# kylegrover/raymarch-algo-compare

Measured on AMD Instinct MI355X. Metric: Mrays/sec (mean iters/ray alongside), 1920x1080 Mandelbulb/Standard, higher is better.
Workload: dtype f64

## Files before the change

raymarch_algo_compare_amd/csrc/rm_capi.hip:

```cpp
#include <hip/hip_runtime.h>
#include <dlfcn.h>
#include <link.h>
#include <rccl/rccl.h>

#include <algorithm>
#include <cstdarg>
#include <cstdio>
#include <cstdlib>
#include <cstring>
#include <map>
#include <memory>
#include <mutex>
#include <optional>
#include <string>
#include <vector>

#include "../../include/rm_hip.h"
#include "rm_kernels.h"
#include "rm_launch_plan.h"
#include "rm_pipeline.h"
#include "rm_scene_program.h"
#include "rm_interval.h"
#include "rm_interval_catalogue.h"
#include "rm_segment.h"
// ... 89 lines not shown
        if (p) (void)hipFree(p);
        p = nullptr; cap = 0;
        hipError_t e = hipMalloc(&p, bytes);
        if (e != hipSuccess) return fail(RM_E_HIP, "hipMalloc(%zu) failed: %s", bytes, hipGetErrorString(e));
        cap = bytes;
        return RM_OK;
    }
    void release()
    {
        if (p) (void)hipFree(p);
        p = nullptr; cap = 0;
    }
};

void release_all(Buf* owner)
{
    for (Buf* b = owner; b; b = b->next) b->release();
}
Buf* g_workspace_bufs = nullptr;
Buf* g_comm_bufs = nullptr;
struct WsBuf : Buf { WsBuf() : Buf(g_workspace_bufs) {} };
struct CommBuf : Buf { CommBuf() : Buf(g_comm_bufs) {} };

struct Session {
    bool ready = false;
    int device = -1;
    hipStream_t stream = nullptr;
    hipDeviceProp_t prop;
    bool stats_ready = false;
    long long cost_key[10] = { -1 };
    bool cost_valid = false;
    hipEvent_t ev[2 * RM_MAX_TIMED];
    bool events = false;
    bool tracing = false;
    size_t trace_pix = 0;
    unsigned long long trace_t0 = 0;
    long long corder_key[12] = { -1 };
    bool corder_valid = false;
    bool pass_timing = false;
    hipEvent_t pev[RM_MAX_PASSES + 1];
    bool pev_ready = false;
    int pass_count = 0;
    bool last_was_pipeline = false;
    const unsigned long long* last_stats = nullptr;
    float long_marks[4] = { 0.f, 0.f, 0.f, 0.f };
    float last_push_ms = 0.f, last_pop_ms = 0.f;
    uint32_t generation = 0;
    struct QueueKey { int stride = 0; int writer = 0; size_t used = 0; } qkey[rm::kQueues];
    hipEvent_t frame_ev = nullptr;
    hipStream_t frame_stream = nullptr;
    bool frame_ev_valid = false;
    hipStream_t team_stream = nullptr;
    hipEvent_t split_ev[2] = { nullptr, nullptr };
};

struct State : Session {
    WsBuf stats, depth, iters, hit, traw, fs, bvar, evals, tcost, torder, queue[rm::kQueues];
    WsBuf in[2], out[4];
    WsBuf bstats;
    WsBuf ivprog;
    WsBuf ctl;
    WsBuf busy;
    WsBuf trace, trace_start, trace_detach;
    WsBuf ccost, corder;
    WsBuf ssim_depth, ssim_normal, ssim_color, ssim_hit;
    WsBuf ssim_ref, ssim_part, ssim_ssd, ssim_out;
    WsBuf score_depth, score_normal, score_hit, score_caps;
    WsBuf score_band, score_keys, score_small, score_part;
    WsBuf cap_out[5], cap_cams;
} g;

std::mutex g_mu;

struct Program {
    std::unique_ptr<rm::ProgramImage> img;
    void* dev = nullptr;
    double lipschitz = 1.0;
    bool ext = false;
};
std::mutex g_prog_mu;
std::map<int32_t, Program> g_programs;
int32_t g_next_program = RM_SCENE_PROGRAM_BASE;

bool is_program_id(int id) { return id >= RM_SCENE_PROGRAM_BASE; }

const rm::SceneLaunchers* program_launchers(bool ext)
{
#if defined(RM_DEV_STRATEGIES)
    if (ext) return rm::scene_launchers_program_ext ? rm::scene_launchers_program_ext() : nullptr;
    return rm::scene_launchers_program ? rm::scene_launchers_program() : nullptr;
#else
    return ext ? rm::scene_launchers_program_ext() : rm::scene_launchers_program();
#endif
}

bool program_exists(int id, bool* ext = nullptr)
{
    std::lock_guard<std::mutex> lk(g_prog_mu);
    auto it = g_programs.find(id);
    if (it == g_programs.end()) return false;
    if (ext) *ext = it->second.ext;
    return true;
}

const rm::SceneLaunchers* launchers(int id)
{
// ... 189 lines not shown
    if (d->tile_rows != 0 && d->tile_rows != 4 && d->tile_rows != 1) return fail(RM_E_BAD_ARG, "tile_rows must be 0, 4 or 1");
    if (d->tile_order_mode < 0 || d->tile_order_mode > 4) return fail(RM_E_BAD_ARG, "tile_order_mode must be 0 .. 4");
    if (d->eval_mode < 0 || d->eval_mode > 2) return fail(RM_E_BAD_ARG, "eval_mode must be 0, 1 or 2");
    if (d->resume_mode < 0 || d->resume_mode > 3) return fail(RM_E_BAD_ARG, "resume_mode must be 0..3");
    if (d->resume_grid < 0) return fail(RM_E_BAD_ARG, "negative resume_grid");
    if (d->pipeline < 0 || d->pipeline > 2) return fail(RM_E_BAD_ARG, "pipeline must be 0, 1 or 2");
    if (d->pipeline_form < 0 || d->pipeline_form > 3) return fail(RM_E_BAD_ARG, "pipeline_form must be 0 .. 3");
    if (d->team_grid < 0 || d->queue_first < 0 || d->queue_first > 3 || d->team_steal < 0 || d->team_steal > 2 ||
        d->queue_refill_min < 0 || d->queue_refill_min > 64 || d->queue_retry < 0 || d->team_retry < 0 || d->age_priority < 0)
        return fail(RM_E_BAD_ARG, "bad single-launch tuning field");
    if (d->exit_backlog < 0 || d->late_teams > 65536) return fail(RM_E_BAD_ARG, "bad late-team field");
    if (d->keep_busy > (1 << 20)) return fail(RM_E_BAD_ARG, "keep_busy out of range");
    if (d->early_handover > (1 << 20)) return fail(RM_E_BAD_ARG, "early_handover out of range");
    if (d->early_trips < 0 || d->early_trips > 64) return fail(RM_E_BAD_ARG, "early_trips out of range");
    if (d->band_rows < 0 || d->band_stride < 0 || d->band_offset < 0) return fail(RM_E_BAD_ARG, "negative band parameter");
    if (d->band_rows > 0 && d->band_stride > 1) {
        const int th = d->tile_rows ? d->tile_rows : 4;
        if (d->band_rows % th) return fail(RM_E_BAD_ARG, "band_rows must be a multiple of the tile height %d", th);
        if (d->band_offset >= d->band_stride) return fail(RM_E_BAD_ARG, "band_offset must be < band_stride");
        if (d->rows > 0) {
            const long long y = d->rows - 1;
            const long long last = d->row0 + ((y / d->band_rows) * d->band_stride + d->band_offset) * d->band_rows + y % d->band_rows;
            if (last >= d->height) return fail(RM_E_BAD_DIMS, "band-cyclic slice maps row %lld beyond height %d", last, d->height);
        }
    }
    return RM_OK;
}

rm::MarchCfg to_cfg(const RmMarchConfig& m)
{
    rm::MarchCfg c;
    c.hit_threshold = m.hit_threshold;
    c.max_distance = m.max_distance;
    c.lipschitz = m.lipschitz;
    c.max_iterations = m.max_iterations;
    c.full = m.full ? 1 : 0;
    c.prm = rm::default_strat_params();
    if (m.use_params) {
        static_assert(sizeof(RmStrategyParams) == sizeof(rm::StratParams), "RmStrategyParams and rm::StratParams must match");
        memcpy(&c.prm, &m.params, sizeof c.prm);
    }
    return c;
}

rm::LaunchPlan plan_for(const RmFrameDesc* d, int batch_frames = 0, const RmMarchConfig* configs = nullptr)
{
    const rm::SceneLaunchers* const sc = launchers(d->scene_id);
    const int strategy = d->strategy_id;
    rm::DeviceFacts f;
    f.cus = g.prop.multiProcessorCount;
    f.has_teams = sc->has_teams;
    f.has_resume_team = sc->resume_team != nullptr;
    f.entry_bytes = sc->entry_bytes(strategy);
    f.per_cu = [sc, strategy](rm::OccKernel k, int , int interleave, int batch) {
        int n = 0;
        const hipError_t e = k == rm::OccKernel::pipeline ? sc->occupancy_pipeline(strategy, interleave, batch, &n)
                                                          : sc->occupancy(strategy, interleave, batch, &n);
        return e == hipSuccess ? n : 0;
    };
    return rm::plan_launch(*d, f, batch_frames, configs);
}

rm::CameraParams camera_of(const double* cam14)
{
    rm::CameraParams c;
    for (int i = 0; i < 14; ++i) c.v[i] = cam14[i];
    return c;
}

int make_args(const RmFrameDesc* d, const rm::LaunchPlan& p, float* depth, int32_t* iters, uint8_t* hit, double* traw, double* fs,
              long long* bvar, unsigned long long* stats, rm::KernelArgs* a)
{
    memset(a, 0, sizeof *a);
    if (int rc = scene_data(d->scene_id, &a->scene_data)) return rc;
    a->single.cam = camera_of(d->cam);
    a->single.cfg = to_cfg(d->march);
    a->frames = nullptr;
    a->nframes = 1;
    a->full = d->march.full ? 1 : 0;
    a->width = d->width; a->height = d->height; a->row0 = d->row0; a->rows = d->rows;
    a->tiles_x = p.tiles_x;
    a->tiles_y = p.tiles_y;
    a->tiles_per_frame = a->tiles_x * a->tiles_y;
    a->tile_h = p.tile_h;
    a->refill_min = p.refill_min;
    a->hist_bins = rm::kHistBins;
    a->interleave = p.interleave;
    a->age_prio = d->age_priority > 0 ? d->age_priority : 0;
    if (d->band_rows > 0 && d->band_stride > 1) {
        a->band_rows = d->band_rows; a->band_stride = d->band_stride; a->band_offset = d->band_offset;
    }
    a->depth = depth; a->iters = iters; a->hit = hit; a->t_raw = traw; a->final_sdf = fs;
    a->block_var = bvar; a->stats = stats;
    a->fused_reduce = p.fused_reduce;
    if (p.park[0] > 0) {
        a->suspend_after = p.park[0];
        a->suspend_queue = 0;
    }
    if (p.single) {
        a->team_wgs = p.team_wgs;
        a->producer_waves = p.producer_waves;
        a->late_team_first = p.late_team_first;
        a->early_exit_wgs = p.early_exit_wgs;
        a->exit_backlog = p.exit_backlog;
        a->keep_busy = p.keep_busy;
        a->early_trips = p.early_trips;
        a->early_handover = p.early_handover;
        a->suspend_after2 = p.suspend_after2;
        a->q0_detach = p.q0_detach;
        a->q0_first = p.q0_first;
        a->q0_refill_min = p.q0_refill_min;
        a->q0_retry = p.q0_retry;
        a->team_retry = p.team_retry;
        a->team_steal = p.team_steal;
        a->max_spins = p.max_spins;
        a->team_prio = p.team_prio;
    }
    return RM_OK;
}

__global__ __launch_bounds__(1024) void order_tiles_kernel(const int32_t* __restrict__ cost, int32_t* __restrict__ order, int n)
{
    constexpr int BINS = 1024;
    __shared__ int hist[BINS];
    for (int b = threadIdx.x; b < BINS; b += blockDim.x) hist[b] = 0;
    __syncthreads();
    for (int i = threadIdx.x; i < n; i += blockDim.x) atomicAdd(&hist[min(max(cost[i], 0), BINS - 1)], 1);
    __syncthreads();
    if (threadIdx.x == 0) {
        int run = 0;
        for (int b = BINS - 1; b >= 0; --b) { const int c = hist[b]; hist[b] = run; run += c; }
    }
    __syncthreads();
    for (int i = threadIdx.x; i < n; i += blockDim.x) {
        const int pos = atomicAdd(&hist[min(max(cost[i], 0), BINS - 1)], 1);
        order[pos] = i;
    }
}

__global__ void center_cost_kernel(int32_t* __restrict__ cost, int tiles_x, int tiles_y, int nframes, int tile_h, int width, int height,
                                   int row0, int band_rows, int band_stride, int band_offset, float xweight)
{
    const int t = blockIdx.x * blockDim.x + threadIdx.x;
    if (t >= tiles_x * tiles_y * nframes) return;
    const int tf = t % (tiles_x * tiles_y);
    const int tx = tf % tiles_x, ty = tf / tiles_x;
    const int y0 = ty * tile_h;
    const int gy = band_rows > 0 ? row0 + ((y0 / band_rows) * band_stride + band_offset) * band_rows + (y0 % band_rows) : row0 + y0;
    const float cx = (tx * 64 + 32 - 0.5f * width) / (0.5f * height);
    const float cy = (gy + 0.5f * tile_h - 0.5f * height) / (0.5f * height);
    const float r = sqrtf(xweight * cx * cx + cy * cy);
    cost[t] = max(0, 1023 - (int)(r * 256.0f));
}

__global__ void block_var_kernel(const int32_t* __restrict__ iters, int width, int rows, int nframes,
                                 long long* __restrict__ out)
{
    const int bw = width >> 3, bh = rows >> 2;
    const long long n = (long long)bw * bh * nframes;
    const long long b = (long long)blockIdx.x * blockDim.x + threadIdx.x;
    if (b >= n) return;
    const int f = (int)(b / ((long long)bw * bh));
    const int r = (int)(b - (long long)f * bw * bh);
    const int by = r / bw, bx = r - by * bw;
    const int32_t* p = iters + (size_t)f * (size_t)rows * (size_t)width + (size_t)(by * 4) * (size_t)width + (size_t)(bx * 8);
    long long S = 0, Q = 0;
#pragma unroll
    for (int y = 0; y < 4; ++y)
#pragma unroll
// ... 447 lines not shown

}

extern "C" {

const char* rm_last_error(void) { return g_err; }
int rm_num_scenes(void) { return RM_NUM_SCENES; }

int rm_scene_program_create(const RmSceneOp* ops, int32_t nops, double lipschitz, int32_t* scene_id)
{
    if (!scene_id) return fail(RM_E_BAD_ARG, "scene_id is NULL");
    if (!(lipschitz > 0.0) || !(lipschitz - lipschitz == 0.0)) return fail(RM_E_BAD_ARG, "lipschitz must be finite and > 0");
    std::unique_ptr<rm::ProgramImage> img(new rm::ProgramImage());
    char why[256];
    if (!rm::program_encode(ops, nops, img.get(), why, sizeof why)) return fail(RM_E_BAD_ARG, "scene program: %s", why);
    std::lock_guard<std::mutex> lk(g_prog_mu);
    if (g_next_program == INT32_MAX) return fail(RM_E_BAD_ARG, "scene program ids exhausted");
    const int32_t id = g_next_program++;
    Program& p = g_programs[id];
    p.ext = rm::program_has_ext(*img);
    p.img = std::move(img);
    p.lipschitz = lipschitz;
    *scene_id = id;
    return RM_OK;
}

int rm_scene_program_destroy(int32_t scene_id)
{
    std::lock_guard<std::mutex> lk(g_mu);
    void* dev = nullptr;
    {
        std::lock_guard<std::mutex> lp(g_prog_mu);
        auto it = g_programs.find(scene_id);
        if (it == g_programs.end()) return no_such_program(scene_id);
        dev = it->second.dev;
        g_programs.erase(it);
    }
    if (dev) {
        if (g.ready) (void)hipSetDevice(g.device);
        HIP_TRY(hipFree(dev));
    }
    return RM_OK;
}
int rm_num_strategies(void) { return RM_NUM_STRATEGIES; }

void rm_default_strategy_params(RmStrategyParams* out)
{
    if (!out) return;
    const rm::StratParams p = rm::default_strat_params();
    memcpy(out, &p, sizeof *out);
}
size_t rm_stats_device_bytes(void) { return kStatsBytes; }

int rm_init(int device_id)
{
    std::lock_guard<std::mutex> lk(g_mu);
    if (g.ready && g.device == device_id) return RM_OK;
    if (g.ready) return fail(RM_E_BAD_ARG, "already initialised on device %d; call rm_shutdown() first", g.device);
    int n = 0;
    hipError_t e = hipGetDeviceCount(&n);
    if (e != hipSuccess || n <= 0)
        return fail(RM_E_NO_DEVICE, "no HIP device available (%s)", e == hipSuccess ? "count = 0" : hipGetErrorString(e));
    if (device_id < 0 || device_id >= n) return fail(RM_E_NO_DEVICE, "device %d out of range (have %d)", device_id, n);
    HIP_TRY(hipSetDevice(device_id));
    HIP_TRY(hipGetDeviceProperties(&g.prop, device_id));
    if (strncmp(g.prop.gcnArchName, "gfx950", 6) != 0)
        return fail(RM_E_NO_DEVICE, "device %d is %s; this library carries gfx950 code only", device_id, g.prop.gcnArchName);
    HIP_TRY(hipStreamCreateWithFlags(&g.stream, hipStreamNonBlocking));
    int rc = g.stats.ensure(kStatsBytes);
    if (rc) return rc;
    g.device = device_id;
    g.ready = true;
    return RM_OK;
}

void rm_shutdown(void)
{
    std::lock_guard<std::mutex> lk(g_mu);
    if (!g.ready) return;
    (void)hipSetDevice(g.device);
    (void)hipStreamSynchronize(g.stream);
    if (g.team_stream) {
        (void)hipStreamSynchronize(g.team_stream);
        for (auto& e : g.split_ev) (void)hipEventDestroy(e);
        (void)hipStreamDestroy(g.team_stream);
    }
    for (void* s : g_own_streams) {
        (void)hipStreamSynchronize((hipStream_t)s);
        (void)hipStreamDestroy((hipStream_t)s);
    }
    g_own_streams.clear();
    g_seen_streams.clear();
    release_all(g_workspace_bufs);
    if (g.frame_ev_valid) (void)hipEventDestroy(g.frame_ev);
    if (g.events) for (auto& e : g.ev) (void)hipEventDestroy(e);
    if (g.pev_ready) for (auto& e : g.pev) (void)hipEventDestroy(e);
    {
        std::lock_guard<std::mutex> lp(g_prog_mu);
        for (auto& kv : g_programs)
            if (kv.second.dev) {
                (void)hipFree(kv.second.dev);
                kv.second.dev = nullptr;
            }
    }
    (void)hipStreamDestroy(g.stream);
    static_cast<Session&>(g) = Session();
}

int rm_device_info(RmDeviceInfo* out)
{
    int rc = check_ready();
    if (rc) return rc;
    if (!out) return fail(RM_E_BAD_ARG, "out is NULL");
    memset(out, 0, sizeof *out);
    snprintf(out->name, sizeof out->name, "%s", g.prop.name);
    snprintf(out->arch, sizeof out->arch, "%s", g.prop.gcnArchName);
    out->device_id = g.device;
    out->compute_units = g.prop.multiProcessorCount;
    out->clock_mhz = g.prop.clockRate / 1000;
    out->wavefront_size = g.prop.warpSize;
    out->total_mem_bytes = g.prop.totalGlobalMem;
    return RM_OK;
}
// ... 1190 lines not shown
```

raymarch_algo_compare_amd/csrc/rm_kernels.h:

```cpp
#pragma once

#define RM_TABLES_IN_LDS 1

#include <hip/hip_runtime.h>
#include <stdint.h>
#include <type_traits>

#include "rm_camera.h"
#include "rm_capture.h"
#include "rm_scenes.h"
#include "rm_shape.h"
#include "rm_strategies.h"

namespace rm {

constexpr int kHistBins = 544;
constexpr int kStatsHead = 24;
constexpr int kStatsWords = kStatsHead + kHistBins;
constexpr int kQueues = 2;
constexpr int kStatsParts = 64;
constexpr int kStatsBlocks = 1 + kStatsParts;

struct FrameParams {
    CameraParams cam;
// ... 20 lines not shown
}


struct KernelArgs {
    FrameParams single;
    const FrameParams* frames;
    int32_t nframes;
    int32_t tiles_per_frame;
    int32_t full;
    int32_t width, height, row0, rows;
    int32_t tiles_x, tiles_y;
    int32_t tile_h;
    int32_t refill_min;
    int32_t interleave;
    int32_t hist_bins;
    int32_t band_rows, band_stride, band_offset;
    float* depth;
    int32_t* iters;
    uint8_t* hit;
    double* t_raw;
    int32_t* evals;
    double* final_sdf;
    int32_t raw_outputs;
    int32_t fused_reduce;
    long long* block_var;
    unsigned long long* stats;
    int32_t suspend_after, suspend_queue, queue_cap, queue_stride;
    unsigned char* queue[kQueues];
    const int32_t* tile_order;
    int32_t* tile_cost;
    unsigned long long* ctl;
    int32_t team_wgs, producer_waves;
    uint32_t generation;
    int32_t suspend_after2;
    int32_t q0_first;
    int32_t q0_detach;
    int32_t q0_refill_min;
    int32_t q0_retry;
    int32_t team_retry;
    int32_t team_steal;
    int32_t max_spins;
    int32_t team_prio;
    int32_t age_prio;
    int32_t marks;
    int32_t early_handover;
    int32_t early_trips;
    int32_t keep_busy;
    int32_t late_team_first, early_exit_wgs, exit_backlog;
    uint32_t* trace;
    uint32_t trace_cap;
    uint32_t* trace_start;
    uint32_t* trace_detach;
    const void* scene_data;
};

__device__ __forceinline__ int lane_id() { return (int)__builtin_amdgcn_mbcnt_hi(~0u, __builtin_amdgcn_mbcnt_lo(~0u, 0u)); }
__device__ __forceinline__ int rank_in_mask(unsigned long long m)
{
    return (int)__builtin_amdgcn_mbcnt_hi((unsigned)(m >> 32), __builtin_amdgcn_mbcnt_lo((unsigned)m, 0u));
}

__device__ __forceinline__ void store_raw(const KernelArgs& a, uint32_t gi, const Result& r, int nev)
{
    if (a.t_raw) a.t_raw[gi] = r.t;
#ifdef RM_DEV_STAMP
    if (a.evals) a.evals[gi] = (int)(__builtin_amdgcn_s_memrealtime() & 0x3fffffffull);
#else
    if (a.final_sdf) a.final_sdf[gi] = r.final_sdf;
    if (a.evals) a.evals[gi] = nev;
#endif
}

__device__ __forceinline__ void keep_busy_until(const unsigned long long* done, unsigned long long target, int burst)
{
    const unsigned long long t0 = __builtin_amdgcn_s_memrealtime();
    float f0 = (float)lane_id(), f1 = f0 + 1.0f, f2 = f0 + 2.0f, f3 = f0 + 3.0f;
    for (;;) {
        unsigned long long n = 0;
        if (lane_id() == 0) n = __hip_atomic_load(done, __ATOMIC_RELAXED, __HIP_MEMORY_SCOPE_AGENT);
        n = (unsigned long long)(unsigned)__builtin_amdgcn_readfirstlane((int)n);
        if (n >= target || __builtin_amdgcn_s_memrealtime() - t0 > 3000000ull) break;
        for (int i = 0; i < burst; ++i) {
            f0 = __builtin_fmaf(f0, 1.0000001f, 1e-9f); f1 = __builtin_fmaf(f1, 1.0000001f, 1e-9f);
            f2 = __builtin_fmaf(f2, 1.0000001f, 1e-9f); f3 = __builtin_fmaf(f3, 1.0000001f, 1e-9f);
        }
    }
    asm volatile("" :: "v"(f0), "v"(f1), "v"(f2), "v"(f3));
}

template <class T>
__device__ __forceinline__ void copy_table(T* dst, const T* src, int n)
{
    for (int i = threadIdx.x; i < n; i += blockDim.x) dst[i] = src[i];
}

template <class Scene, class = void>
struct SceneLaunchData : std::false_type {};
template <class Scene>
struct SceneLaunchData<Scene, decltype((void)Scene::kLaunchData)> : std::integral_constant<bool, Scene::kLaunchData> {};
template <class Scene>
__device__ __forceinline__ void rm_load_scene_data(const void* data)
{
    if constexpr (SceneLaunchData<Scene>::value) Scene::load(data);
}

template <class Scene>
// ... 874 lines not shown
```

raymarch_algo_compare_amd/csrc/rm_launch_plan.h:

```cpp
#pragma once

#include <algorithm>
#include <functional>

#include "../../include/rm_hip.h"
#include "rm_shape.h"

namespace rm {

enum class OccKernel { render, pipeline };

struct DeviceFacts {
    int cus = 0;
    bool has_teams = false;
    bool has_resume_team = false;
    int entry_bytes = 0;
    std::function<int(OccKernel kernel, int tile_h, int interleave, int batch)> per_cu;
};

struct LaunchPlan {
    const char* refuse = nullptr;
    int nframes = 1;
    bool batch = false;
    int march_frame = -1;
    long long rays = 0;
    int tile_h = 4, tiles_x = 0, tiles_y = 0;
    int refill_min = 0, interleave = 0;
    int mode = 1;
    int park[2] = { 0, 0 };
    bool single = false;
    int fused_reduce = 0;
    int tile_order = 0;
    int static_order = 0;
    int render_grid = 0;
    int queue_entry_bytes = 0;
    int team_wgs = 0, producer_waves = 0, late_team_first = 0, early_exit_wgs = 0, exit_backlog = 0, keep_busy = 0;
    int early_trips = 0, early_handover = 0, suspend_after2 = 0;
    int q0_detach = 0, q0_first = 0, q0_refill_min = 0, q0_retry = 0, team_retry = 0, team_steal = 0, team_prio = 0, max_spins = 0;
    int pipeline_grid = 0;
    int resume_grid = 0, resume_refill_min = 0, pass_keep_busy = 0, team_pass_grid = 0;
    bool pass_team[2] = { false, false };
};

inline int grid_per_cu(int reached) { return reached <= 0 ? 2 : std::min(reached, 3); }

inline int resolve_keep_busy(const RmFrameDesc& d) { return d.keep_busy > 0 ? d.keep_busy : (d.keep_busy == 0 ? 256 : 0); }

inline int pipeline_mode(const RmFrameDesc& d, long long rays, int max_iterations)
{
    if (d.scene_id >= RM_SCENE_PROGRAM_BASE) return 1;
    if (d.pipeline != 0) return d.pipeline;
    return (d.scene_id == 10 && rays <= 24000000ll && max_iterations > 128) ? 2 : 1;
}

inline void suspend_levels(const RmFrameDesc& d, long long rays, int mode, int max_iterations, int* park)
{
    const bool strat_ok = d.strategy_id != 6 && d.strategy_id != 7;
    const bool long_budget = rays <= 16000000ll && max_iterations > 128;
    const bool dflt = d.scene_id == 10 && strat_ok && long_budget;
    const int two = (d.strategy_id == 10 || d.strategy_id == 8) ? 2 : 1;
    const int d0 = (rays <= 3000000ll ? 32 : 48) / two, d1 = (rays <= 3000000ll ? 128 : 192) / two;
    park[0] = d.suspend_after[0] > 0 ? d.suspend_after[0] : (d.suspend_after[0] == 0 && dflt ? d0 : 0);
    park[1] = d.suspend_after[1] > 0 ? d.suspend_after[1] : (d.suspend_after[1] == 0 && dflt && d.suspend_after[0] == 0 ? d1 : 0);
    if ((d.scene_id == 1 || d.scene_id == 13) && d.strategy_id != 7 && d.suspend_after[0] == 0 && long_budget) park[0] = 128;
    if ((d.scene_id == 14 || d.scene_id == 15) && strat_ok && d.strategy_id != 9 && d.suspend_after[0] == 0 && long_budget)
        park[0] = 16 / two;
    if (mode == 2 && d.scene_id == 10 && max_iterations > 128) {
        const bool small = rays <= 3000000ll && d.strategy_id != 10 && d.tile_order_mode != 1;
        const bool ordered = rays <= 3000000ll && d.strategy_id != 10 && d.tile_order_mode == 1;
        if (d.suspend_after[0] == 0) park[0] = small ? 16 : (ordered ? 24 : 32);
        if (d.suspend_after[1] == 0 && d.suspend_after[0] == 0) park[1] = small ? 48 : (ordered ? 56 : 64);
    }
    if (park[0] == 0) park[1] = 0;
    if (park[1] > 0 && park[1] <= park[0]) park[1] = 0;
}

inline int default_tile_order(const RmFrameDesc& d, int nframes)
{
    if (nframes > 1) return d.scene_id == 10 ? 2 : 3;
    switch (d.scene_id) {
        case 1: case 13: return 3;
        case 3: case 5: case 12: return 4;
        default: return 2;
    }
}

inline void plan_single_launch(const RmFrameDesc& d, const DeviceFacts& dev, LaunchPlan& p)
{
    const bool teams = dev.has_teams && p.park[1] > 0 && d.resume_mode != 1;
    const int per_cu = grid_per_cu(dev.per_cu(OccKernel::pipeline, p.tile_h, p.interleave, p.batch ? 1 : 0));
    const long long resident = (long long)dev.cus * per_cu;
    const long long ntiles = (long long)p.tiles_x * p.tiles_y * p.nframes;
    const long long rays = p.rays;
    long long team_wgs = 0;
    if (teams) {
        long long share16 = rays <= 1000000ll ? 7 : (rays <= 3000000ll ? 6 : 3);
        if (rays > 600000ll && rays <= 1000000ll) share16 = d.strategy_id == 4 ? 4 : 5;
        if (d.tile_order_mode == 1 && rays <= 3000000ll) share16 = 7;
        if (p.nframes > 1 && rays > 3000000ll) share16 = 4;
        if (d.strategy_id == 6 || d.strategy_id == 9) share16 = d.tile_order_mode == 1 ? 4 : 3;
        if (d.strategy_id == 7 && d.tile_order_mode == 1) share16 = 4;
        team_wgs = d.team_grid > 0 ? d.team_grid : std::max<long long>(1, resident * share16 / 16);
        team_wgs = std::min<long long>(team_wgs, std::max<long long>(1, resident / 2));
    }
    long long late = 0;
    const bool detach_mode = d.queue_first == 3 || (d.queue_first == 0 && teams);
    if (teams && detach_mode && d.grid_waves == 0) {
        if (d.late_teams > 0) late = d.late_teams;
    }
    const long long want_pw = d.grid_waves > 0 ? d.grid_waves : resident * kPipeWaves;
    long long pure = (std::min<long long>(want_pw, ntiles) + kPipeWaves - 1) / kPipeWaves;
    pure = std::max<long long>(1, std::min<long long>(pure, resident - team_wgs));
    late = std::min<long long>(late, std::max<long long>(0, pure - 1));
    p.team_wgs = (int)team_wgs;
    p.producer_waves = (int)(pure * kPipeWaves);
    p.late_team_first = (int)(team_wgs + pure);
    p.early_exit_wgs = (int)late;
    p.pipeline_grid = (int)(pure + late + team_wgs);
    p.exit_backlog = d.exit_backlog > 0 ? d.exit_backlog : 64;
    p.keep_busy = (teams && late == 0) ? resolve_keep_busy(d) : 0;
    p.early_trips = d.early_trips > 0 ? d.early_trips : 8;
    const bool eh_default = d.strategy_id != 6 && d.strategy_id != 7 && d.strategy_id != 9;
    p.early_handover = (teams && detach_mode)
        ? (d.early_handover > 0 ? d.early_handover : (d.early_handover == 0 && eh_default ? std::max(1, p.park[0]) : 0)) : 0;
    p.suspend_after2 = teams ? p.park[1] : 0;
    p.q0_detach = detach_mode ? 1 : 0;
    p.q0_first = (d.queue_first == 0 || d.queue_first == 1) ? 1 : 0;
    p.q0_refill_min = d.queue_refill_min > 0 ? d.queue_refill_min : 16;
    p.q0_retry = d.queue_retry > 0 ? d.queue_retry : 16;
    p.team_retry = d.team_retry > 0 ? d.team_retry : 8;
    p.team_steal = (d.team_steal == 0 || d.team_steal == 1) ? 1 : 0;
    p.team_prio = 3;
    p.max_spins = 50000;
}

inline void plan_passes(const RmFrameDesc& d, const DeviceFacts& dev, LaunchPlan& p)
{
    p.resume_refill_min = 16;
    p.resume_grid = d.resume_grid > 0 ? d.resume_grid : std::min(p.render_grid, dev.cus);
    const bool team = dev.has_resume_team && d.resume_mode != 1;
    p.pass_keep_busy = team ? resolve_keep_busy(d) : 0;
    p.team_pass_grid = p.pass_keep_busy > 0 ? 2 * p.resume_grid : p.resume_grid;
    p.pass_team[0] = team && (p.park[1] == 0 || d.resume_mode == 3);
    p.pass_team[1] = team;
}

inline LaunchPlan plan_launch(const RmFrameDesc& d, const DeviceFacts& dev, int batch_frames = 0, const RmMarchConfig* configs = nullptr)
{
    LaunchPlan p;
    p.batch = batch_frames > 0;
    p.nframes = p.batch ? batch_frames : 1;
    int max_iterations = d.march.max_iterations;
    if (p.batch && configs) {
        p.march_frame = 0;
        for (int f = 1; f < p.nframes; ++f)
            if (configs[f].max_iterations > configs[p.march_frame].max_iterations) p.march_frame = f;
        max_iterations = configs[p.march_frame].max_iterations;
    }
    p.rays = (long long)d.rows * d.width * p.nframes;
    p.tile_h = d.tile_rows ? d.tile_rows : 4;
    p.tiles_x = (d.width + kTileW - 1) / kTileW;
    p.tiles_y = (d.rows + p.tile_h - 1) / p.tile_h;
    int refill_default = 8;
    switch (d.scene_id) { case 0: case 2: case 3: case 4: case 6: case 18: case 19: refill_default = 16; break; default: break; }
    p.refill_min = (d.refill_min > 0 && d.refill_min <= 64) ? d.refill_min : refill_default;
    p.interleave = d.eval_mode == 2 || (d.eval_mode == 0 && d.scene_id == 10);

    p.mode = pipeline_mode(d, p.rays, max_iterations);
    suspend_levels(d, p.rays, p.mode, max_iterations, p.park);
    p.single = p.park[0] > 0 && p.mode == 2;
    p.fused_reduce = (p.park[0] == 0 && p.nframes == 1 && d.rows > 0) ? 1 : 0;
    if (d.tile_rows == 1 && !(p.single && dev.has_teams))
        p.refuse = "tile_rows = 1 exists for the single launch (pipeline = 2 with suspension) of scenes with a team form";
    if (p.single && dev.has_teams && (d.tile_rows == 1 || (d.tile_rows == 0 && d.tile_order_mode == 1))) {
        p.tile_h = 1;
        p.tiles_y = d.rows;
    }
    p.static_order = default_tile_order(d, p.nframes);
    p.tile_order = d.tile_order_mode != 0 ? d.tile_order_mode : p.static_order;
    if (p.park[0] > 0) p.queue_entry_bytes = dev.entry_bytes;

    if (p.single) {
        plan_single_launch(d, dev, p);
        return p;
    }
    const long long frame_tiles = (long long)p.tiles_x * p.tiles_y;
// ... 15 lines not shown
```

raymarch_algo_compare_amd/csrc/rm_pipeline.h:

```cpp
#pragma once

#include "rm_kernels.h"

namespace rm {

constexpr int kCtlStride = 16;
constexpr int kCTile = 0;
constexpr int kCReserved = 1;
constexpr int kCTaken = 3;
constexpr int kCFreshDone = 5;
constexpr int kCProdExited = 6;
constexpr int kCLeft = 7;
constexpr int kCLateStarted = 8;
constexpr int kCTeamDone = 9;
constexpr int kCtlWords = 10 * kCtlStride;
__device__ __forceinline__ unsigned long long* ctl(const KernelArgs& a, int k) { return a.ctl + k * kCtlStride; }
constexpr int kWMarkStart = 13;
constexpr int kWMarkFresh = 14;
constexpr int kWMarkProd = 15;
constexpr int kWMarkTiles = 17;
constexpr int kWMarkPush = 18;
constexpr int kWMarkPop = 19;
constexpr int kWLongPushMax = 20;
constexpr int kWLongTeamMax = 21;
constexpr int kWLongTeamMin = 22;
constexpr int kWLongPushMin = 23;
constexpr int kLongRay = 500;
constexpr int kWError = 16;
constexpr int kMaxReadyPolls = 4000000;
constexpr unsigned long long kMaxTeamWaitTicks = 3000000000ull;

__device__ __forceinline__ unsigned long long ld_relaxed(const unsigned long long* p)
{
    return __hip_atomic_load(p, __ATOMIC_RELAXED, __HIP_MEMORY_SCOPE_AGENT);
}
__device__ __forceinline__ void add_after_drain(unsigned long long* p, unsigned long long v)
{
    asm volatile("s_waitcnt vmcnt(0)" ::: "memory");
    __hip_atomic_fetch_add(p, v, __ATOMIC_RELAXED, __HIP_MEMORY_SCOPE_AGENT);
}
__device__ __forceinline__ unsigned long long realtime() { return __builtin_amdgcn_s_memrealtime(); }

__device__ __forceinline__ long long q_available(const KernelArgs& a, int q)
{
    unsigned long long R = ld_relaxed(ctl(a, kCReserved + q));
    if (R > (unsigned long long)a.queue_cap) R = (unsigned long long)a.queue_cap;
    const unsigned long long T = ld_relaxed(ctl(a, kCTaken + q));
    return (long long)R - (long long)T;
}

__device__ __forceinline__ int q_claim_lane0(const KernelArgs& a, int q, int want, unsigned int& base)
{
    unsigned long long R = ld_relaxed(ctl(a, kCReserved + q));
    if (R > (unsigned long long)a.queue_cap) R = (unsigned long long)a.queue_cap;
    unsigned long long T = ld_relaxed(ctl(a, kCTaken + q));
    for (int tries = 0; tries < 8 && T < R; ++tries) {
        const unsigned long long nt = (T + (unsigned long long)want < R) ? T + (unsigned long long)want : R;
        if (__hip_atomic_compare_exchange_strong(ctl(a, kCTaken + q), &T, nt, __ATOMIC_RELAXED, __ATOMIC_RELAXED,
                                                 __HIP_MEMORY_SCOPE_AGENT)) {
            base = (unsigned int)T;
            return (int)(nt - T);
        }
    }
    return 0;
}

template <class Strat>
__device__ __forceinline__ bool q_wait_ready(const KernelArgs& a, int q, bool mine, unsigned int idx)
// ... 93 lines not shown
};

__device__ __forceinline__ void store_direct(const KernelArgs& a, uint32_t gi, const Result& r, int nev, WaveAcc& acc,
                                             unsigned int* s_hist)
{
    const int it = r.iters, h = r.hit;
    a.depth[gi] = h ? (float)r.t : 0.0f;
    a.iters[gi] = it;
    a.hit[gi] = (uint8_t)h;
    if (a.raw_outputs) store_raw(a, gi, r, nev);
    acc.evals += (unsigned)nev;
    acc.add(it, h);
    atomicAdd(&s_hist[min(it, a.hist_bins - 1)], 1u);
    if (a.tile_cost) {
        const uint32_t frame_elems = (uint32_t)a.rows * (uint32_t)a.width;
        const uint32_t frame = gi / frame_elems;
        const uint32_t pix = gi - frame * frame_elems;
        const uint32_t y = pix / (uint32_t)a.width, x = pix - y * (uint32_t)a.width;
        atomicMax(&a.tile_cost[frame * (uint32_t)a.tiles_per_frame + (y / (uint32_t)a.tile_h) * (uint32_t)a.tiles_x + (x >> 6)], it);
    }
}

template <class Scene, class E>
__device__ __forceinline__ auto early_handover(const KernelArgs& a, const E& ev, int i) -> decltype(Scene::eval_trips(ev), bool())
{
    return a.early_handover > 0 && i >= a.early_handover && Scene::eval_trips(ev) >= a.early_trips;
}
template <class Scene>
__device__ __forceinline__ bool early_handover(const KernelArgs&, const NoEval&, int) { return false; }
template <class Scene, class E>
__device__ __forceinline__ bool early_handover(const KernelArgs&, const E&, long) { return false; }

template <class Scene, class Strat, bool BATCH>
__device__ __forceinline__ void pipe_team_role(const KernelArgs& a, const KernelArgs& ar, PipeTeamLds& L, const int part, const int lane)
{
    WaveAcc acc;
    if (a.team_prio >= 3) __builtin_amdgcn_s_setprio(3);
    else if (a.team_prio == 2) __builtin_amdgcn_s_setprio(2);
    else if (a.team_prio == 1) __builtin_amdgcn_s_setprio(1);
    bool active = false;
    uint32_t my_gi = 0;
    uint32_t my_push = 0;
    uint32_t my_pop = 0, nev_pop = 0;
    int nev = 0;
    vec3 origin = v3(0.0, 0.0, 0.0), dir = v3(0.0, 0.0, 0.0);
    MarchCfg lane_cfg = a.single.cfg;
    if constexpr (!BATCH) pin_cfg(lane_cfg);
    const MarchCfg& cfg = lane_cfg;
    Strat s;
    typename Scene::Eval ev;
    int turn = 0;
    int since_try = 0;
    unsigned long long idle_since = 0;

    for (;;) {
        const unsigned long long idle = __ballot(!active);
        const int nidle = __popcll(idle);
        const bool look = nidle == 64 || (nidle >= a.refill_min && since_try >= a.team_retry);
        if (look) {
            since_try = 0;
            if (part == 0) {
                unsigned int base = 0, done = 0;
                int q = 1, cnt = 0;
                if (lane == 0) {
                    cnt = q_claim_lane0(ar, 1, nidle, base);
                    if (cnt == 0 && ar.team_steal) { q = 0; cnt = q_claim_lane0(ar, 0, nidle, base); }
                    if (cnt == 0 && nidle == 64) {
                        const unsigned long long ex = ld_relaxed(ctl(ar, kCProdExited));
                        if (ex >= (unsigned long long)ar.producer_waves && q_available(ar, 1) <= 0 && q_available(ar, 0) <= 0) done = 1;
                        const unsigned long long now = realtime();
                        if (idle_since == 0) idle_since = now;
                        if (!done && now - idle_since > kMaxTeamWaitTicks) { atomicMax(&ar.stats[kWError], 2ull); done = 1; }
                    } else if (cnt > 0) {
                        idle_since = 0;
                        if (ar.marks && q == 1) atomicMax(&ar.stats[kWMarkPop], realtime());
                    }
                }
                cnt = __builtin_amdgcn_readfirstlane(cnt);
                q = __builtin_amdgcn_readfirstlane(q);
                base = (unsigned int)__builtin_amdgcn_readfirstlane((int)base);
                unsigned long long okm = 0;
                if (cnt > 0) {
                    const int rank = rank_in_mask(idle);
                    const bool want = !active && rank < cnt;
                    const bool got = q_wait_ready<Strat>(ar, q, want, base + (unsigned int)rank);
                    okm = __ballot(want && got);
                }
                if (lane == 0) {
                    L.base = base; L.count = (unsigned int)cnt; L.queue = (unsigned int)q; L.done = done;
                    L.ok_lo = (unsigned int)okm; L.ok_hi = (unsigned int)(okm >> 32);
                }
            }
            __syncthreads();
            const unsigned int base = L.base, cnt = L.count, q = L.queue, done = L.done;
            const unsigned long long okm = ((unsigned long long)L.ok_hi << 32) | (unsigned long long)L.ok_lo;
            __syncthreads();
            if (done) break;
            if (cnt > 0) {
                if (part != 0) __builtin_amdgcn_fence(__ATOMIC_ACQUIRE, "agent");
                const int rank = rank_in_mask(idle);
                const bool mine = ((okm >> lane) & 1ull) != 0;
                if (mine) {
                    const QEntry<Strat>* const e = (const QEntry<Strat>*)ar.queue[q] + (base + (unsigned int)rank);
                    my_gi = e->gi;
                    nev = (int)e->nev;
                    s = e->s;
                    my_push = e->pad;
                    if (ar.trace) { my_pop = (uint32_t)(realtime() - ~ld_relaxed(&ar.stats[kWMarkStart])); nev_pop = (uint32_t)nev; }
                    uint32_t frame; int x, gy;
                    element_pixel(ar, my_gi, frame, x, gy);
                    if constexpr (BATCH) {
                        const FrameParams& fp = ar.frames[frame];
                        camera_ray(fp.cam, ar.width, ar.height, x, gy, origin, dir);
                        lane_cfg = fp.cfg;
                        lane_cfg.full = ar.full;
                    } else {
                        camera_ray(ar.single.cam, ar.width, ar.height, x, gy, origin, dir);
                    }
                    active = true;
// ... 38 lines not shown
        }
    }
    unsigned long long* const spart = stats_part(ar.stats);
    if (part == 0) acc.flush(spart);
    __syncthreads();
    for (int b = part * 64 + lane; b < kHistBins; b += 64 * kTeam) {
        const unsigned int c = L.hist[b];
        if (c) atomicAdd(&spart[kStatsHead + b], (unsigned long long)c);
    }
    if (part == 0 && lane == 0) __hip_atomic_fetch_add(ctl(ar, kCTeamDone), 1ull, __ATOMIC_RELAXED, __HIP_MEMORY_SCOPE_AGENT);
}

template <class Scene, class Strat, int TILE_H, bool INTERLEAVE, bool BATCH, bool TEAM_ROLE, bool SPLIT>
__device__ __forceinline__ void pipeline_body(const KernelArgs& ka, const KernelArgs& a)
{
    static_assert(!INTERLEAVE || SceneIterative<Scene>::value, "INTERLEAVE needs Scene::Eval");
    constexpr bool TEAMS = SceneIterative<Scene>::value;
    static_assert(TEAMS || !TEAM_ROLE, "team workgroups need a team form");
    constexpr int TILE_PIX = kTileW * TILE_H;
    using Entry = QEntry<Strat>;
    using PLds = PipeProducerLds<TILE_PIX>;
    constexpr size_t kRoleBytes = (!TEAM_ROLE || sizeof(PLds) > sizeof(PipeTeamLds)) ? sizeof(PLds) : sizeof(PipeTeamLds);
    __shared__ __attribute__((aligned(16))) unsigned char s_role[kRoleBytes];
    __shared__ unsigned int s_hist[kHistBins];
    __shared__ unsigned int s_leave;

    const int lane = lane_id();
    const int wave = (int)(threadIdx.x >> 6);
    for (int b = threadIdx.x; b < kHistBins; b += blockDim.x) s_hist[b] = 0u;
    if (threadIdx.x == 0) s_leave = 0u;
    rm_load_tables<Scene>();
    __syncthreads();
    if (a.marks && threadIdx.x == 0) atomicMax(&a.stats[kWMarkStart], ~realtime());

    WaveAcc acc;
    const bool late_team = TEAM_ROLE && (int)blockIdx.x >= a.late_team_first;
    const bool team_wg = TEAM_ROLE && ((int)blockIdx.x < a.team_wgs || late_team);
    if (late_team && threadIdx.x == 0) __hip_atomic_fetch_add(ctl(a, kCLateStarted), 1ull, __ATOMIC_RELAXED, __HIP_MEMORY_SCOPE_AGENT);
    constexpr int kRole[8] = { 0, 1, 2, -1, -1, -1, -1, -1 };
    const int wave_role = !team_wg ? -2 : kRole[wave & 7];
    const bool team_role = team_wg && wave_role >= 0;
    if (team_wg) {
        PipeTeamLds& T = *reinterpret_cast<PipeTeamLds*>(s_role);
        for (int b = threadIdx.x; b < kHistBins; b += blockDim.x) T.hist[b] = 0u;
        if (threadIdx.x == 0) { T.base = T.count = T.queue = T.done = 0u; T.ok_lo = T.ok_hi = 0u; }
        __syncthreads();
    }

    if constexpr (TEAM_ROLE) {
    if (team_wg && wave_role == -1) return;
    if (team_role) {
        const int team = wave_role / kTeam;
        const int part = wave_role % kTeam;
        pipe_team_role<Scene, Strat, BATCH>(a, a, reinterpret_cast<PipeTeamLds*>(s_role)[team], part, lane);
        return;
    }
    }

    PLds& L = *reinterpret_cast<PLds*>(s_role);
    float (*const s_depth)[TILE_PIX] = L.depth[wave];
    uint32_t (*const s_ih)[TILE_PIX] = L.ih[wave];
    const int ntiles = ka.tiles_per_frame * ka.nframes;
    const int team_wgs = TEAM_ROLE ? a.team_wgs : 0;
    int pwave = ((int)blockIdx.x - team_wgs) * kPipeWaves + wave;
    if constexpr (SPLIT) pwave = __builtin_amdgcn_readfirstlane(pwave);
    const int park0 = ka.suspend_after;
    const int park1 = (TEAMS && ka.team_wgs > 0) ? ka.suspend_after2 : 0;
    const bool queues = park0 > 0;
    const bool detach = SPLIT || a.q0_detach != 0;
    const bool may_leave = !SPLIT && TEAMS && detach && park1 > 0 && ((int)blockIdx.x - team_wgs) < a.early_exit_wgs;
    bool leaving = false;

    int slot_tile[kSlots], slot_out[kSlots];
#pragma unroll
    for (int k = 0; k < kSlots; ++k) { slot_tile[k] = -1; slot_out[k] = 0; }
    int cur = 0;
    int pool_next = TILE_PIX;
    bool more_tiles = true;
    bool first_tile = true;
    TileGeom cg = { 0, 0, 0, 0, 0, 0, 0 };

    bool active = false;
    bool resumed = false;
    bool nopark = false;
    int my_slot = 0, my_pix = 0;
    uint32_t my_gi = 0;
    int nev = 0;
    vec3 origin = v3(0.0, 0.0, 0.0), dir = v3(0.0, 0.0, 0.0);
    MarchCfg lane_cfg = a.single.cfg;
    if constexpr (!BATCH) pin_cfg(lane_cfg);
    const MarchCfg& cfg = lane_cfg;
    int raw_out = a.raw_outputs;
    pin_lane(raw_out);
    Strat s;
    typename EvalOf<Scene, INTERLEAVE>::type ev;
    bool ready = false;
    bool dirty = true;
    bool fresh_reported = false;
    int spins = 0;
    int since_look = 0;

    for (;;) {
        if (dirty) {
        dirty = false;
        since_look = 0;
#pragma unroll
        for (int k = 0; k < kSlots; ++k) {
            const bool pool_done = (k != cur) || pool_next >= TILE_PIX;
            if (slot_tile[k] >= 0 && slot_out[k] == 0 && pool_done) {
                wave_lds_fence();
                const TileGeom g = tile_geom<TILE_H>(a, slot_tile[k]);
                const int gx = g.x0 + lane;
                const bool col_ok = lane < g.tw;
                long long bs = 0, bq = 0;
                const bool want_bv = a.block_var != nullptr;
                float* o_depth = a.depth; int32_t* o_iters = a.iters; uint8_t* o_hit = a.hit;
                pin_lane(o_depth); pin_lane(o_iters); pin_lane(o_hit);
#pragma unroll
                for (int r = 0; r < TILE_H; ++r) {
                    if (r < g.th && col_ok) {
// ... 236 lines not shown
                    store_direct(a, my_gi, s.res, nev, acc, s_hist);
                    freed = true;
                } else {
                    fin = true;
                    s_depth[my_slot][my_pix] = s.res.hit ? (float)s.res.t : 0.0f;
                    s_ih[my_slot][my_pix] = (uint32_t)s.res.iters | ((uint32_t)s.res.hit << 31);
                    if (raw_out) store_raw(a, my_gi, s.res, nev);
                    acc.evals += (unsigned)nev;
                }
            } else if (!nopark && ((!resumed && park0 > 0 && s.i >= park0) || (resumed && park1 > 0 && (s.i >= park1 || leaving || early_handover<Scene>(a, ev, s.i))))) {
                park = true;
            } else if constexpr (INTERLEAVE) {
                ready = Scene::begin(ev, origin + dir * s.te);
            }
        }
        if (queues && __any(park)) {
            bool p0 = park && !resumed;
            const bool p1 = park && resumed;
            bool parked = false;
            if (detach) {
                if (p0) {
                    if (a.trace_detach) a.trace_detach[my_gi] = (uint32_t)realtime();
                    s_ih[my_slot][my_pix] = kSuspended;
                    fin = true;
                    resumed = true;
                    park = false;
                    if constexpr (INTERLEAVE) ready = Scene::begin(ev, origin + dir * s.te);
                }
                p0 = false;
            }
            if (__any(p0)) parked = q_push<Strat>(a, 0, p0, my_gi, s, nev);
            if (__any(p1)) parked = q_push<Strat>(a, 1, p1, my_gi, s, nev) || parked;
            if (parked) {
                if (!resumed) { s_ih[my_slot][my_pix] = kSuspended; fin = true; }
                else freed = true;
                active = false;
            } else if (park) {
                nopark = true;
                if constexpr (INTERLEAVE) ready = Scene::begin(ev, origin + dir * s.te);
            }
        }
        if (__any(fin)) {
#pragma unroll
            for (int k = 0; k < kSlots; ++k) slot_out[k] -= __popcll(__ballot(fin && my_slot == k));
            dirty = true;
        }
        if (__any(freed)) dirty = true;
        }
        if (queues && !detach && ++since_look >= a.q0_retry) {
            since_look = 0;
            if (__popcll(__ballot(!active)) >= a.q0_refill_min) dirty = true;
        }
        if constexpr (INTERLEAVE) {
            if (active && !ready) ready = Scene::trip(ev);
        }
    }

    unsigned long long* const part = stats_part(a.stats);
    acc.flush(part);
    if (queues && lane == 0) {
        if (!fresh_reported) add_after_drain(ctl(a, kCFreshDone), 1ull);
        add_after_drain(ctl(a, kCProdExited), 1ull);
        if (a.marks) atomicMax(&a.stats[kWMarkProd], realtime());
    }
    __syncthreads();
    for (int b = threadIdx.x; b < kHistBins; b += blockDim.x) {
        const unsigned int c = s_hist[b];
        if (c) atomicAdd(&part[kStatsHead + b], (unsigned long long)c);
    }
    if (TEAMS && a.keep_busy > 0 && !team_wg && a.team_wgs > 0) keep_busy_until(ctl(a, kCTeamDone), (unsigned long long)a.team_wgs, a.keep_busy);
}

template <class Scene, class Strat, int TILE_H, bool INTERLEAVE, bool BATCH>
__global__ __launch_bounds__(64 * kPipeWaves, 2) void pipeline_kernel(const KernelArgs a)
{
    pipeline_body<Scene, Strat, TILE_H, INTERLEAVE, BATCH, SceneIterative<Scene>::value, false>(a, a);
}

template <class Scene, class Strat, int TILE_H, bool INTERLEAVE, bool BATCH>
__global__ __launch_bounds__(64 * kPipeWaves, 2) void pipeline_producer_kernel(const KernelArgs a)
{
    __shared__ KernelArgs s_args;
    if (threadIdx.x == 0) s_args = a;
    pipeline_body<Scene, Strat, TILE_H, INTERLEAVE, BATCH, false, true>(a, s_args);
}

template <class Scene, class Strat, bool BATCH>
__global__ __launch_bounds__(64 * kTeam) void pipeline_team_kernel(const KernelArgs a)
{
    __shared__ PipeTeamLds T;
    __shared__ KernelArgs s_args;
    if (threadIdx.x == 0) s_args = a;
    for (int b = threadIdx.x; b < kHistBins; b += blockDim.x) T.hist[b] = 0u;
    if (threadIdx.x == 0) { T.base = T.count = T.queue = T.done = 0u; T.ok_lo = T.ok_hi = 0u; }
    rm_load_tables<Scene>();
    __syncthreads();
    if (a.marks && threadIdx.x == 0) atomicMax(&a.stats[kWMarkStart], ~realtime());
    pipe_team_role<Scene, Strat, BATCH>(a, s_args, T, (int)(threadIdx.x >> 6), lane_id());
}

}
```

Measured before the change: 277.8.

## Add env-gated extra trips for resumed rays and team queue hold heuristic

Adds two new scheduling knobs, struck_trips and hold_after, both defaulting to zero and settable only through environment variables. struck_trips lets resumed rays in interleaved mode run several extra trip steps in one loop iteration, and hold_after lets team waves skip claiming new work when they hold old rays and idle teams need the queue, using a new global idle-team counter. With the defaults, the visible changes are that pipeline_kernel now copies KernelArgs into LDS and reads kernel args from there, the team role gets those LDS args, and pwave is always made wave-uniform. These default-path edits slightly shift register and scalar-load pressure, and the trip loop adds a small amount of control flow.

```diff
diff --git a/raymarch_algo_compare_amd/csrc/rm_capi.hip b/raymarch_algo_compare_amd/csrc/rm_capi.hip
--- a/raymarch_algo_compare_amd/csrc/rm_capi.hip
+++ b/raymarch_algo_compare_amd/csrc/rm_capi.hip
@@ -165,6 +165,7 @@
     bool frame_ev_valid = false;
     hipStream_t team_stream = nullptr;
     hipEvent_t split_ev[2] = { nullptr, nullptr };
+    int struck_trips_override = -1, hold_after_override = -1;
 };
 
 struct State : Session {
@@ -460,7 +461,9 @@
     f.has_teams = sc->has_teams;
     f.has_resume_team = sc->resume_team != nullptr;
     f.entry_bytes = sc->entry_bytes(strategy);
-    f.per_cu = [sc, strategy](rm::OccKernel k, int , int interleave, int batch) {
+    f.struck_trips_override = g.struck_trips_override;
+    f.hold_after_override = g.hold_after_override;
+    f.per_cu =[sc, strategy](rm::OccKernel k, int , int interleave, int batch) {
         int n = 0;
         const hipError_t e = k == rm::OccKernel::pipeline ? sc->occupancy_pipeline(strategy, interleave, batch, &n)
                                                           : sc->occupancy(strategy, interleave, batch, &n);
@@ -523,6 +526,8 @@
         a->team_steal = p.team_steal;
         a->max_spins = p.max_spins;
         a->team_prio = p.team_prio;
+        a->struck_trips = p.struck_trips;
+        a->hold_after = p.hold_after;
     }
     return RM_OK;
 }
@@ -1076,6 +1081,15 @@
 }
 size_t rm_stats_device_bytes(void) { return kStatsBytes; }
 
+static int env_override(const char* name, long max)
+{
+    const char* const v = getenv(name);
+    if (!v || !*v) return -1;
+    char* end = nullptr;
+    const long n = strtol(v, &end, 10);
+    return (*end == '\0' && n >= 0 && n <= max) ? (int)n : -1;
+}
+
 int rm_init(int device_id)
 {
     std::lock_guard<std::mutex> lk(g_mu);
@@ -1093,6 +1107,8 @@
     HIP_TRY(hipStreamCreateWithFlags(&g.stream, hipStreamNonBlocking));
     int rc = g.stats.ensure(kStatsBytes);
     if (rc) return rc;
+    g.struck_trips_override = env_override("RM_STRUCK_TRIPS", 8);
+    g.hold_after_override = env_override("RM_TEAM_HOLD_AFTER", 65536);
     g.device = device_id;
     g.ready = true;
     return RM_OK;
diff --git a/raymarch_algo_compare_amd/csrc/rm_kernels.h b/raymarch_algo_compare_amd/csrc/rm_kernels.h
--- a/raymarch_algo_compare_amd/csrc/rm_kernels.h
+++ b/raymarch_algo_compare_amd/csrc/rm_kernels.h
@@ -96,6 +96,8 @@
     uint32_t* trace_start;
     uint32_t* trace_detach;
     const void* scene_data;
+    int32_t struck_trips;
+    int32_t hold_after;
 };
 
 __device__ __forceinline__ int lane_id() { return (int)__builtin_amdgcn_mbcnt_hi(~0u, __builtin_amdgcn_mbcnt_lo(~0u, 0u)); }
diff --git a/raymarch_algo_compare_amd/csrc/rm_launch_plan.h b/raymarch_algo_compare_amd/csrc/rm_launch_plan.h
--- a/raymarch_algo_compare_amd/csrc/rm_launch_plan.h
+++ b/raymarch_algo_compare_amd/csrc/rm_launch_plan.h
@@ -16,6 +16,7 @@
     bool has_resume_team = false;
     int entry_bytes = 0;
     std::function<int(OccKernel kernel, int tile_h, int interleave, int batch)> per_cu;
+    int struck_trips_override = -1, hold_after_override = -1;
 };
 
 struct LaunchPlan {
@@ -40,6 +41,7 @@
     int pipeline_grid = 0;
     int resume_grid = 0, resume_refill_min = 0, pass_keep_busy = 0, team_pass_grid = 0;
     bool pass_team[2] = { false, false };
+    int struck_trips = 0, hold_after = 0;
 };
 
 inline int grid_per_cu(int reached) { return reached <= 0 ? 2 : std::min(reached, 3); }
@@ -132,6 +134,11 @@
     p.team_steal = (d.team_steal == 0 || d.team_steal == 1) ? 1 : 0;
     p.team_prio = 3;
     p.max_spins = 50000;
+    const bool struck_mech = p.interleave != 0 && p.park[0] > 0;
+    const int struck_default = 0;
+    p.struck_trips = !struck_mech ? 0 : (dev.struck_trips_override >= 0 ? dev.struck_trips_override : struck_default);
+    const int hold_default = 0;
+    p.hold_after = !teams ? 0 : (dev.hold_after_override >= 0 ? dev.hold_after_override : hold_default);
 }
 
 inline void plan_passes(const RmFrameDesc& d, const DeviceFacts& dev, LaunchPlan& p)
diff --git a/raymarch_algo_compare_amd/csrc/rm_pipeline.h b/raymarch_algo_compare_amd/csrc/rm_pipeline.h
--- a/raymarch_algo_compare_amd/csrc/rm_pipeline.h
+++ b/raymarch_algo_compare_amd/csrc/rm_pipeline.h
@@ -13,7 +13,8 @@
 constexpr int kCLeft = 7;
 constexpr int kCLateStarted = 8;
 constexpr int kCTeamDone = 9;
-constexpr int kCtlWords = 10 * kCtlStride;
+constexpr int kCIdleTeams = 10;
+constexpr int kCtlWords = 11 * kCtlStride;
 __device__ __forceinline__ unsigned long long* ctl(const KernelArgs& a, int k) { return a.ctl + k * kCtlStride; }
 constexpr int kWMarkStart = 13;
 constexpr int kWMarkFresh = 14;
@@ -213,6 +214,7 @@
     int turn = 0;
     int since_try = 0;
     unsigned long long idle_since = 0;
+    bool counted_idle = false;
 
     for (;;) {
         const unsigned long long idle = __ballot(!active);
@@ -223,9 +225,18 @@
             if (part == 0) {
                 unsigned int base = 0, done = 0;
                 int q = 1, cnt = 0;
+                const bool old_ray = ar.hold_after > 0 && __any(active && nev >= ar.hold_after);
                 if (lane == 0) {
-                    cnt = q_claim_lane0(ar, 1, nidle, base);
-                    if (cnt == 0 && ar.team_steal) { q = 0; cnt = q_claim_lane0(ar, 0, nidle, base); }
+                    bool hold = false;
+                    if (old_ray) hold = q_available(ar, 1) < (long long)ld_relaxed(ctl(ar, kCIdleTeams)) * 64;
+                    if (!hold) {
+                        cnt = q_claim_lane0(ar, 1, nidle, base);
+                        if (cnt == 0 && ar.team_steal) { q = 0; cnt = q_claim_lane0(ar, 0, nidle, base); }
+                    }
+                    if (ar.hold_after > 0 && counted_idle != (cnt == 0 && nidle == 64)) {
+                        counted_idle = !counted_idle;
+                        __hip_atomic_fetch_add(ctl(ar, kCIdleTeams), counted_idle ? 1ull : ~0ull, __ATOMIC_RELAXED, __HIP_MEMORY_SCOPE_AGENT);
+                    }
                     if (cnt == 0 && nidle == 64) {
                         const unsigned long long ex = ld_relaxed(ctl(ar, kCProdExited));
                         if (ex >= (unsigned long long)ar.producer_waves && q_available(ar, 1) <= 0 && q_available(ar, 0) <= 0) done = 1;
@@ -370,7 +381,7 @@
     if (team_role) {
         const int team = wave_role / kTeam;
         const int part = wave_role % kTeam;
-        pipe_team_role<Scene, Strat, BATCH>(a, a, reinterpret_cast<PipeTeamLds*>(s_role)[team], part, lane);
+        pipe_team_role<Scene, Strat, BATCH>(ka, a, reinterpret_cast<PipeTeamLds*>(s_role)[team], part, lane);
         return;
     }
     }
@@ -381,9 +392,10 @@
     const int ntiles = ka.tiles_per_frame * ka.nframes;
     const int team_wgs = TEAM_ROLE ? a.team_wgs : 0;
     int pwave = ((int)blockIdx.x - team_wgs) * kPipeWaves + wave;
-    if constexpr (SPLIT) pwave = __builtin_amdgcn_readfirstlane(pwave);
+    pwave = __builtin_amdgcn_readfirstlane(pwave);
     const int park0 = ka.suspend_after;
     const int park1 = (TEAMS && ka.team_wgs > 0) ? ka.suspend_after2 : 0;
+    const int struck_trips = INTERLEAVE ? ka.struck_trips : 0;
     const bool queues = park0 > 0;
     const bool detach = SPLIT || a.q0_detach != 0;
     const bool may_leave = !SPLIT && TEAMS && detach && park1 > 0 && ((int)blockIdx.x - team_wgs) < a.early_exit_wgs;
@@ -726,7 +738,12 @@
             if (__popcll(__ballot(!active)) >= a.q0_refill_min) dirty = true;
         }
         if constexpr (INTERLEAVE) {
-            if (active && !ready) ready = Scene::trip(ev);
+            bool go = active && !ready;
+            for (int extra = struck_trips;; --extra) {
+                if (go) ready = Scene::trip(ev);
+                go = go && !ready && resumed;
+                if (extra <= 0 || !__any(go)) break;
+            }
         }
     }
 
@@ -748,7 +765,9 @@
 template <class Scene, class Strat, int TILE_H, bool INTERLEAVE, bool BATCH>
 __global__ __launch_bounds__(64 * kPipeWaves, 2) void pipeline_kernel(const KernelArgs a)
 {
-    pipeline_body<Scene, Strat, TILE_H, INTERLEAVE, BATCH, SceneIterative<Scene>::value, false>(a, a);
+    __shared__ KernelArgs s_args;
+    if (threadIdx.x == 0) s_args = a;
+    pipeline_body<Scene, Strat, TILE_H, INTERLEAVE, BATCH, SceneIterative<Scene>::value, false>(a, s_args);
 }
 
 template <class Scene, class Strat, int TILE_H, bool INTERLEAVE, bool BATCH>
```

After: 277.2, median of 2. Within noise of the previous version (-0.2%).
